# second-state/qwen3_asr_rs

Measured on NVIDIA H100. Metric: real-time factor (audio-sec/wall-sec) Qwen3-ASR-0.6B 30s clips, higher is better.
Workload: dtype f32 (bf16 weights, fp32-exact activations)

## Files before the change

qwen3_asr_rs_b200/csrc/attention_f32.cu:

```cuda
#include "internal.h"

namespace asrb {

namespace af32 {

static constexpr int QT = 32, KT = 64, THREADS = 128, PS = KT + 4;

template <int HD, bool OFF>
__global__ void __launch_bounds__(THREADS, 2) attn_f32_kernel(AttnParams p) {
    constexpr int NG = HD / 64;
    extern __shared__ __align__(16) float sm[];
    float* Qt = sm;
    float* Kt = Qt + HD * QT;
    float* Vs = Kt + HD * KT;
    float* Ps = Vs + KT * HD;
    const int seg = blockIdx.z, h = blockIdx.y;
    const int q0 = p.seg_q0[seg], len = p.seg_len[seg];
    const int pos0 = OFF ? p.seg_pos0[seg] : 0;
    const int nqt = (len + QT - 1) / QT;
    const int gkv = h / p.group;
    const int tid = threadIdx.x, tx = tid & 15, ty = tid >> 4;
    const float* kbase; const float* vbase;
    if (p.keys_in_rows) {
        kbase = p.k + (size_t)q0 * p.ldk + (size_t)gkv * p.head_stride;
        vbase = p.v + (size_t)q0 * p.ldk + (size_t)gkv * p.head_stride;
    } else {
        kbase = p.k + (size_t)seg * p.seg_stride + (size_t)gkv * p.head_stride;
        vbase = p.v + (size_t)seg * p.seg_stride + (size_t)gkv * p.head_stride;
    }
    const int npass = p.causal ? 2 : 1;
    for (int pass = 0; pass < npass; ++pass) {
    const int qtile = pass == 0 ? (int)blockIdx.x : nqt - 1 - (int)blockIdx.x;
    if (qtile >= nqt || qtile < 0 || (p.causal && pass == 0 && 2 * qtile >= nqt) || (pass == 1 && qtile <= (int)blockIdx.x)) continue;
    const int qt0 = qtile * QT;
    __syncthreads();
    {
        constexpr int NQ = QT * (HD / 4) / THREADS;
        float4 qr[NQ];
#pragma unroll
        for (int u = 0; u < NQ; ++u) {
            const int idx = tid + u * THREADS, r = idx % QT, c4 = idx / QT;
            qr[u] = make_float4(0.f, 0.f, 0.f, 0.f);
            if (qt0 + r < len) qr[u] = *reinterpret_cast<const float4*>(p.q + (size_t)(q0 + qt0 + r) * p.ldq + (size_t)h * HD + c4 * 4);
        }
#pragma unroll
        for (int u = 0; u < NQ; ++u) {
            const int idx = tid + u * THREADS, r = idx % QT, c4 = idx / QT;
            Qt[(c4 * 4 + 0) * QT + r] = qr[u].x; Qt[(c4 * 4 + 1) * QT + r] = qr[u].y;
            Qt[(c4 * 4 + 2) * QT + r] = qr[u].z; Qt[(c4 * 4 + 3) * QT + r] = qr[u].w;
        }
    }
    float o[4][NG][4];
#pragma unroll
    for (int i = 0; i < 4; ++i)
#pragma unroll
        for (int gq = 0; gq < NG; ++gq) { o[i][gq][0] = o[i][gq][1] = o[i][gq][2] = o[i][gq][3] = 0.f; }
    float m_run[4], l_run[4];
#pragma unroll
    for (int i = 0; i < 4; ++i) { m_run[i] = -INFINITY; l_run[i] = 0.f; }
    const int kend = p.causal ? pos0 + min(len, qt0 + QT) : len;
    const float div = sqrtf((float)HD);

    for (int kt0 = 0; kt0 < kend; kt0 += KT) {
        __syncthreads();
        constexpr int NLD = KT * (HD / 4) / THREADS, LB = 8;
        static_assert(NLD % LB == 0, "tile load batches");
#pragma unroll
        for (int b0 = 0; b0 < NLD; b0 += LB) {
            float4 kr[LB];
#pragma unroll
            for (int u = 0; u < LB; ++u) {
                const int idx = tid + (b0 + u) * THREADS, r = idx % KT, c4 = idx / KT;
                kr[u] = make_float4(0.f, 0.f, 0.f, 0.f);
                if (kt0 + r < kend) kr[u] = *reinterpret_cast<const float4*>(kbase + (size_t)(kt0 + r) * p.ldk + c4 * 4);
            }
#pragma unroll
            for (int u = 0; u < LB; ++u) {
                const int idx = tid + (b0 + u) * THREADS, r = idx % KT, c4 = idx / KT;
                Kt[(c4 * 4 + 0) * KT + r] = kr[u].x; Kt[(c4 * 4 + 1) * KT + r] = kr[u].y;
                Kt[(c4 * 4 + 2) * KT + r] = kr[u].z; Kt[(c4 * 4 + 3) * KT + r] = kr[u].w;
            }
        }
#pragma unroll
        for (int b0 = 0; b0 < NLD; b0 += LB) {
            float4 vr[LB];
#pragma unroll
            for (int u = 0; u < LB; ++u) {
                const int idx = tid + (b0 + u) * THREADS, r = idx / (HD / 4), c4 = idx - r * (HD / 4);
                vr[u] = make_float4(0.f, 0.f, 0.f, 0.f);
                if (kt0 + r < kend) vr[u] = *reinterpret_cast<const float4*>(vbase + (size_t)(kt0 + r) * p.ldk + c4 * 4);
            }
#pragma unroll
            for (int u = 0; u < LB; ++u) {
                const int idx = tid + (b0 + u) * THREADS, r = idx / (HD / 4), c4 = idx - r * (HD / 4);
                *reinterpret_cast<float4*>(Vs + r * HD + c4 * 4) = vr[u];
            }
        }
        __syncthreads();
        float s[4][4];
#pragma unroll
        for (int i = 0; i < 4; ++i) { s[i][0] = s[i][1] = s[i][2] = s[i][3] = 0.f; }
#pragma unroll 8
        for (int d = 0; d < HD; ++d) {
            const float4 a = *reinterpret_cast<const float4*>(Qt + d * QT + ty * 4);
            const float4 b = *reinterpret_cast<const float4*>(Kt + d * KT + tx * 4);
            s[0][0] = fmaf(a.x, b.x, s[0][0]); s[0][1] = fmaf(a.x, b.y, s[0][1]); s[0][2] = fmaf(a.x, b.z, s[0][2]); s[0][3] = fmaf(a.x, b.w, s[0][3]);
            s[1][0] = fmaf(a.y, b.x, s[1][0]); s[1][1] = fmaf(a.y, b.y, s[1][1]); s[1][2] = fmaf(a.y, b.z, s[1][2]); s[1][3] = fmaf(a.y, b.w, s[1][3]);
            s[2][0] = fmaf(a.z, b.x, s[2][0]); s[2][1] = fmaf(a.z, b.y, s[2][1]); s[2][2] = fmaf(a.z, b.z, s[2][2]); s[2][3] = fmaf(a.z, b.w, s[2][3]);
            s[3][0] = fmaf(a.w, b.x, s[3][0]); s[3][1] = fmaf(a.w, b.y, s[3][1]); s[3][2] = fmaf(a.w, b.z, s[3][2]); s[3][3] = fmaf(a.w, b.w, s[3][3]);
        }
#pragma unroll
        for (int i = 0; i < 4; ++i) {
            const int r = qt0 + ty * 4 + i;
            float tmax = -INFINITY;
#pragma unroll
            for (int j = 0; j < 4; ++j) {
                const int col = kt0 + tx * 4 + j;
                const bool valid = (r < len) && (col < pos0 + len) && (!p.causal || col <= pos0 + r);
                const float v = valid ? s[i][j] / div : -INFINITY;
                s[i][j] = v;
                tmax = fmaxf(tmax, v);
            }
#pragma unroll
            for (int off = 1; off < 16; off <<= 1) tmax = fmaxf(tmax, __shfl_xor_sync(0xffffffffu, tmax, off));
            const float m_new = fmaxf(m_run[i], tmax);
            const float corr = (m_new == -INFINITY) ? 1.f : expf(m_run[i] - m_new);
            m_run[i] = m_new;
            float psum = 0.f;
            float4 pv;
            pv.x = (m_new == -INFINITY) ? 0.f : expf(s[i][0] - m_new);
            pv.y = (m_new == -INFINITY) ? 0.f : expf(s[i][1] - m_new);
            pv.z = (m_new == -INFINITY) ? 0.f : expf(s[i][2] - m_new);
            pv.w = (m_new == -INFINITY) ? 0.f : expf(s[i][3] - m_new);
            psum = (pv.x + pv.y) + (pv.z + pv.w);
#pragma unroll
            for (int off = 1; off < 16; off <<= 1) psum += __shfl_xor_sync(0xffffffffu, psum, off);
            l_run[i] = l_run[i] * corr + psum;
#pragma unroll
            for (int gq = 0; gq < NG; ++gq) { o[i][gq][0] *= corr; o[i][gq][1] *= corr; o[i][gq][2] *= corr; o[i][gq][3] *= corr; }
            *reinterpret_cast<float4*>(Ps + (ty * 4 + i) * PS + tx * 4) = pv;
        }
        __syncwarp();
#pragma unroll 4
        for (int j = 0; j < KT; ++j) {
            float a[4];
#pragma unroll
            for (int i = 0; i < 4; ++i) a[i] = Ps[(ty * 4 + i) * PS + j];
#pragma unroll
            for (int gq = 0; gq < NG; ++gq) {
                const float4 b = *reinterpret_cast<const float4*>(Vs + j * HD + gq * 64 + tx * 4);
#pragma unroll
                for (int i = 0; i < 4; ++i) {
                    o[i][gq][0] = fmaf(a[i], b.x, o[i][gq][0]); o[i][gq][1] = fmaf(a[i], b.y, o[i][gq][1]);
                    o[i][gq][2] = fmaf(a[i], b.z, o[i][gq][2]); o[i][gq][3] = fmaf(a[i], b.w, o[i][gq][3]);
                }
            }
        }
        __syncwarp();
    }
#pragma unroll
    for (int i = 0; i < 4; ++i) {
        const int r = qt0 + ty * 4 + i;
        if (r >= len) continue;
        const float inv = 1.0f / l_run[i];
        const size_t base = (size_t)(q0 + r) * p.ldo + (size_t)h * HD;
#pragma unroll
        for (int gq = 0; gq < NG; ++gq)
#pragma unroll
            for (int e = 0; e < 4; ++e) store_split3(p.out_s3, p.plane_stride, base + gq * 64 + tx * 4 + e, o[i][gq][e] * inv);
    }
    }
}

template <int HD> static size_t smem_bytes() { return (size_t)(HD * QT + HD * KT + KT * HD + QT * PS) * sizeof(float); }

}

bool launch_attention_f32(const AttnParams& p, int hd, cudaStream_t st) {
    using namespace af32;
    if (p.nseg <= 0 || p.max_len <= 0) return true;
    if ((p.ldq % 4) || (p.ldk % 4) || (p.head_stride % 4) || (p.seg_stride % 4)) return false;
    const int nqt_max = (p.max_len + QT - 1) / QT;
    dim3 grid(p.causal ? (nqt_max + 1) / 2 : nqt_max, p.nheads, p.nseg);
    auto run = [&](auto kern, size_t smem) {
        ASRB_CUDA_CHECK(cudaFuncSetAttribute(kern, cudaFuncAttributeMaxDynamicSharedMemorySize, (int)smem));
        kern<<<grid, THREADS, smem, st>>>(p);
    };
    const bool off = p.seg_pos0 != nullptr;
    if (off && !p.causal) return false;
    if (hd == 64) run(off ? attn_f32_kernel<64, true> : attn_f32_kernel<64, false>, smem_bytes<64>());
    else if (hd == 128) run(off ? attn_f32_kernel<128, true> : attn_f32_kernel<128, false>, smem_bytes<128>());
    else return false;
    ASRB_CUDA_CHECK(cudaGetLastError());
    return true;
}

}
```

qwen3_asr_rs_b200/csrc/common.cuh:

```cuda
#pragma once
#include <cuda_runtime.h>
#include <cuda_bf16.h>
#include <stdint.h>
#include <stdexcept>
#include <string>

namespace asrb {

struct Error : public std::runtime_error {
    int code;
    Error(int c, const std::string& m) : std::runtime_error(m), code(c) {}
};

#define ASRB_CUDA_CHECK(expr)                                                              \
    do {                                                                                   \
        cudaError_t _e = (expr);                                                           \
        if (_e != cudaSuccess)                                                             \
            throw ::asrb::Error(2, std::string(#expr) + " failed: " + cudaGetErrorString(_e) + \
                                       " (" __FILE__ ":" + std::to_string(__LINE__) + ")"); \
    } while (0)

#define ASRB_REQUIRE(cond, code, msg)                                          \
    do {                                                                       \
        if (!(cond)) throw ::asrb::Error((code), std::string(msg));            \
    } while (0)

typedef __nv_bfloat16 bf16;

__device__ __forceinline__ float bf16_bits_to_f32(uint32_t bits16) { return __uint_as_float(bits16 << 16); }
__device__ __forceinline__ float bf16_lo(uint32_t packed) { return __uint_as_float(packed << 16); }
__device__ __forceinline__ float bf16_hi(uint32_t packed) { return __uint_as_float(packed & 0xffff0000u); }

struct Split3 { bf16 hi, mid, lo; };
__device__ __forceinline__ Split3 split3(float x) {
    Split3 s;
    s.hi = __float2bfloat16_rn(x);
    float r = x - __bfloat162float(s.hi);
    s.mid = __float2bfloat16_rn(r);
    r = r - __bfloat162float(s.mid);
    s.lo = __float2bfloat16_rn(r);
    return s;
}
__device__ __forceinline__ void store_split3(bf16* base, size_t plane_stride, size_t idx, float x) {
    Split3 s = split3(x);
    base[idx] = s.hi;
    base[plane_stride + idx] = s.mid;
    base[2 * plane_stride + idx] = s.lo;
}
__device__ __forceinline__ float load_split3(const bf16* base, size_t plane_stride, size_t idx, int nplanes) {
    float v = __bfloat162float(base[idx]);
    if (nplanes > 1) v += __bfloat162float(base[plane_stride + idx]);
    if (nplanes > 2) v += __bfloat162float(base[2 * plane_stride + idx]);
    return v;
}

__device__ __forceinline__ float gelu_erf(float x) {
    return 0.5f * x * (1.0f + erff(x * 0.70710678118654752440f));
}
__device__ __forceinline__ float silu(float x) { return x / (1.0f + expf(-x)); }

__device__ __forceinline__ float warp_sum(float v) {
#pragma unroll
    for (int o = 16; o > 0; o >>= 1) v += __shfl_xor_sync(0xffffffffu, v, o);
    return v;
}
__device__ __forceinline__ float warp_max(float v) {
#pragma unroll
    for (int o = 16; o > 0; o >>= 1) v = fmaxf(v, __shfl_xor_sync(0xffffffffu, v, o));
    return v;
}
__device__ __forceinline__ float block_sum(float v, float* scratch) {
    int lane = threadIdx.x & 31, w = threadIdx.x >> 5, nw = (blockDim.x + 31) >> 5;
    v = warp_sum(v);
    __syncthreads();
    if (lane == 0) scratch[w] = v;
    __syncthreads();
    float r = (lane < nw) ? scratch[lane] : 0.f;
    r = warp_sum(r);
    return r;
}
__device__ __forceinline__ float block_max(float v, float* scratch) {
    int lane = threadIdx.x & 31, w = threadIdx.x >> 5, nw = (blockDim.x + 31) >> 5;
    v = warp_max(v);
    __syncthreads();
    if (lane == 0) scratch[w] = v;
    __syncthreads();
    float r = (lane < nw) ? scratch[lane] : -INFINITY;
    r = warp_max(r);
    return r;
}

__device__ __forceinline__ float lse_rescale(float s, float m, float M) { return m == M ? s : s * expf(m - M); }
__device__ __forceinline__ void lse_fold(float v, int row, float& best_v, int& best_i, float& best_s) {
    if (v > best_v) { best_s = lse_rescale(best_s, best_v, v) + 1.f; best_v = v; best_i = row; }
    else best_s += expf(v - best_v);
}
__device__ __forceinline__ float lse_merge(float m, float s, float om, float os) {
    const float M = fmaxf(m, om);
    return lse_rescale(s, m, M) + lse_rescale(os, om, M);
}

constexpr int TK_MAX = 8;
struct TopK { float v[TK_MAX]; int i[TK_MAX]; };
__device__ __forceinline__ bool tk_before(float a, int ai, float b, int bi) { return a > b || (a == b && ai < bi); }
__device__ __forceinline__ void tk_init(TopK& t) {
#pragma unroll
    for (int j = 0; j < TK_MAX; ++j) { t.v[j] = -INFINITY; t.i[j] = 0x7fffffff; }
}
__device__ __forceinline__ void tk_insert(TopK& t, float v, int row) {
    if (!tk_before(v, row, t.v[TK_MAX - 1], t.i[TK_MAX - 1])) return;
#pragma unroll
    for (int j = 0; j < TK_MAX; ++j)
        if (tk_before(v, row, t.v[j], t.i[j])) { const float tv = t.v[j]; const int ti = t.i[j]; t.v[j] = v; t.i[j] = row; v = tv; row = ti; }
}
__device__ __forceinline__ void tk_merge(TopK& t, const TopK& u) {
#pragma unroll
    for (int j = 0; j < TK_MAX; ++j)
        if (!tk_before(t.v[j], t.i[j], u.v[TK_MAX - 1 - j], u.i[TK_MAX - 1 - j])) { t.v[j] = u.v[TK_MAX - 1 - j]; t.i[j] = u.i[TK_MAX - 1 - j]; }
#pragma unroll
    for (int d = TK_MAX / 2; d > 0; d >>= 1)
#pragma unroll
        for (int j = 0; j < TK_MAX; ++j)
            if ((j & d) == 0 && tk_before(t.v[j + d], t.i[j + d], t.v[j], t.i[j])) {
                const float tv = t.v[j]; const int ti = t.i[j];
                t.v[j] = t.v[j + d]; t.i[j] = t.i[j + d]; t.v[j + d] = tv; t.i[j + d] = ti;
            }
}
__device__ __forceinline__ void tk_merge_xor(TopK& t, int o) {
    TopK u;
#pragma unroll
    for (int j = 0; j < TK_MAX; ++j) { u.v[j] = __shfl_xor_sync(0xffffffffu, t.v[j], o); u.i[j] = __shfl_xor_sync(0xffffffffu, t.i[j], o); }
    tk_merge(t, u);
}
__device__ __forceinline__ void tk_store(const TopK& t, float* v, int* i) {
#pragma unroll
    for (int j = 0; j < TK_MAX; ++j) { v[j] = t.v[j]; i[j] = t.i[j]; }
}
__device__ __forceinline__ void tk_merge_from(TopK& t, const float* v, const int* i, bool l2) {
    TopK u;
#pragma unroll
    for (int j = 0; j < TK_MAX; ++j) { u.v[j] = l2 ? __ldcg(v + j) : v[j]; u.i[j] = l2 ? __ldcg(i + j) : i[j]; }
    tk_merge(t, u);
}
__device__ __forceinline__ void tk_write(const TopK& t, float lp, int* ids, float* lps) {
#pragma unroll
    for (int j = 0; j < TK_MAX; ++j) { ids[j] = t.i[j]; lps[j] = j == 0 ? lp : (t.v[j] - t.v[0]) + lp; }
}

struct SampleParams {
    float inv_t;
    uint32_t k0, k1;
};
__host__ __device__ __forceinline__ uint32_t philox4x32_10_x0(uint32_t c0, uint32_t c1, uint32_t c2, uint32_t c3, uint32_t k0, uint32_t k1) {
#pragma unroll
    for (int i = 0; i < 10; ++i) {
        if (i > 0) { k0 += 0x9E3779B9u; k1 += 0xBB67AE85u; }
        const uint64_t p0 = (uint64_t)0xD2511F53u * c0, p1 = (uint64_t)0xCD9E8D57u * c2;
        const uint32_t n0 = (uint32_t)(p1 >> 32) ^ c1 ^ k0, n2 = (uint32_t)(p0 >> 32) ^ c3 ^ k1;
        c0 = n0; c1 = (uint32_t)p1; c2 = n2; c3 = (uint32_t)p0;
    }
    return c0;
}
struct Draw {
    float inv_t; uint32_t k0, k1, n, r;
};
__device__ __forceinline__ Draw make_draw(const SampleParams* sp, int n, int r) {
    Draw d; d.inv_t = __ldg(&sp->inv_t); d.k0 = __ldg(&sp->k0); d.k1 = __ldg(&sp->k1); d.n = (uint32_t)n; d.r = (uint32_t)r;
    return d;
}
__device__ __forceinline__ float gumbel_noise(uint32_t x0) {
    const float u = (float)((x0 >> 8) | 1u) * 0x1p-24f;
    return -logf(-logf(u));
}
__device__ __forceinline__ float sample_key(const Draw& d, float l, int v) {
    return fmaf(l, d.inv_t, gumbel_noise(philox4x32_10_x0((uint32_t)v, d.n, d.r, 0u, d.k0, d.k1)));
}
template <bool LOGPROB>
__device__ __forceinline__ void sample_fold(const Draw& d, float l, int row, float& best_v, int& best_i, float& best_s, float& m,
                                            float& sel) {
    const float k = sample_key(d, l, row);
    if (k > best_v) { best_v = k; best_i = row; if constexpr (LOGPROB) sel = l; }
    if constexpr (LOGPROB) {
        if (l > m) { best_s = lse_rescale(best_s, m, l) + 1.f; m = l; }
        else best_s += expf(l - m);
    }
}
template <bool LOGPROB>
__device__ __forceinline__ void sample_merge_xor(int o, float& best_v, int& best_i, float& best_s, float& m, float& sel) {
    const float ov = __shfl_xor_sync(0xffffffffu, best_v, o); const int oi = __shfl_xor_sync(0xffffffffu, best_i, o);
    float osel = 0.f;
    if constexpr (LOGPROB) {
        osel = __shfl_xor_sync(0xffffffffu, sel, o);
        const float om = __shfl_xor_sync(0xffffffffu, m, o);
        best_s = lse_merge(m, best_s, om, __shfl_xor_sync(0xffffffffu, best_s, o));
        m = fmaxf(m, om);
    }
    if (ov > best_v || (ov == best_v && oi < best_i)) { best_v = ov; best_i = oi; if constexpr (LOGPROB) sel = osel; }
}

struct RepParams {
    float theta;
    int ngram;
};
struct RepBits {
    const uint32_t* hist; const uint32_t* ban; int w0; float theta;
};
__device__ __forceinline__ void rep_mark(const int* __restrict__ ids, int n, int N, int lo, int hi, uint32_t* hist,
                                         uint32_t* ban, int t, int nt) {
    const int w0 = lo >> 5;
    for (int i = t; i < n; i += nt) {
        const int v = __ldcg(ids + i);
        if (v >= lo && v < hi) atomicOr(hist + ((v >> 5) - w0), 1u << (v & 31));
        if (N >= 1 && i <= n - N) {
            bool match = true;
            for (int j = 0; j < N - 1 && match; ++j) match = __ldcg(ids + i + j) == __ldcg(ids + n - N + 1 + j);
            if (match) {
                const int u = __ldcg(ids + i + N - 1);
                if (u >= lo && u < hi) atomicOr(ban + ((u >> 5) - w0), 1u << (u & 31));
            }
        }
    }
}
__device__ __forceinline__ bool rep_logit(const RepBits& r, int v, float& l) {
    const int w = (v >> 5) - r.w0;
    const uint32_t bit = 1u << (v & 31);
    if (r.ban[w] & bit) { l = -INFINITY; return false; }
    if (r.hist[w] & bit) l = l < 0.f ? l * r.theta : l / r.theta;
    return true;
}
template <bool REP>
__device__ __forceinline__ bool rep_keep(const RepBits* r, int v, float& l) {
    if constexpr (REP) return rep_logit(*r, v, l);
    else return true;
}

__device__ __host__ __forceinline__ int float_to_ordered(float f) {
#ifdef __CUDA_ARCH__
    int i = __float_as_int(f);
#else
    int i; memcpy(&i, &f, 4);
#endif
    return i >= 0 ? i : i ^ 0x7fffffff;
}
__device__ __forceinline__ float ordered_to_float(int k) {
    int i = k >= 0 ? k : k ^ 0x7fffffff;
    return __int_as_float(i);
}

}
```

qwen3_asr_rs_b200/csrc/elementwise.cu:

```cuda
#include "internal.h"

namespace asrb {

__global__ void conv1_gelu_kernel(const float* __restrict__ mel, const int* __restrict__ chunk_clip,
                                  const int* __restrict__ chunk_f0, const int64_t* __restrict__ foff,
                                  const int64_t* __restrict__ frames, int n_mels, int W, int OH, int OW,
                                  const float* __restrict__ w, const float* __restrict__ bias, int dsh,
                                  int cpad, bf16* __restrict__ out, size_t plane_stride) {
    extern __shared__ float rows[];
    const int chunk = blockIdx.y, oh = blockIdx.x;
    const int clip = chunk_clip[chunk], f0 = chunk_f0[chunk];
    const int F = (int)frames[clip];
    const float* mp = mel + (size_t)n_mels * foff[clip];
    for (int idx = threadIdx.x; idx < 3 * (W + 2); idx += blockDim.x) {
        int kh = idx / (W + 2), wi = idx - kh * (W + 2);
        int h = 2 * oh + kh - 1, wcol = wi - 1;
        float v = 0.f;
        if (h >= 0 && h < n_mels && wcol >= 0 && wcol < W && f0 + wcol < F) v = mp[(size_t)h * F + f0 + wcol];
        rows[idx] = v;
    }
    __syncthreads();
    const int c = threadIdx.x;
    if (c >= dsh) return;
    float wk[9];
#pragma unroll
    for (int i = 0; i < 9; ++i) wk[i] = w[c * 9 + i];
    const float bc = bias ? bias[c] : 0.f;
    const int Hh = OH / 2 + (OH & 1), Wh = (OW + 1) / 2;
    for (int ow = 0; ow < OW; ++ow) {
        float acc = bc;
#pragma unroll
        for (int kh = 0; kh < 3; ++kh)
#pragma unroll
            for (int kw = 0; kw < 3; ++kw) acc = fmaf(wk[kh * 3 + kw], rows[kh * (W + 2) + 2 * ow + kw], acc);
        float v = gelu_erf(acc);
        size_t pos = ((((size_t)chunk * 2 + (oh & 1)) * 2 + (ow & 1)) * Hh + (oh >> 1)) * Wh + (ow >> 1);
        store_split3(out, plane_stride, pos * cpad + c, v);
    }
}

void launch_conv1(const Model& m, const float* mel, const int* d_chunk_clip, const int* d_chunk_f0,
                  const int64_t* d_foff, const int64_t* d_frames, int n_chunks, bf16* out_s3,
                  size_t plane_stride, cudaStream_t st) {
    const Dims& d = m.d;
    int W = d.conv_w[0], OH = d.conv_h[1], OW = d.conv_w[1];
    dim3 grid(OH, n_chunks);
    int threads = ((d.c.downsample_hidden_size + 31) / 32) * 32;
    size_t smem = 3 * (W + 2) * sizeof(float);
    conv1_gelu_kernel<<<grid, threads, smem, st>>>(mel, d_chunk_clip, d_chunk_f0, d_foff, d_frames,
                                                   d.c.num_mel_bins, W, OH, OW, m.conv1_w, m.conv1_b,
                                                   d.c.downsample_hidden_size, d.cpad, out_s3, plane_stride);
    ASRB_CUDA_CHECK(cudaGetLastError());
}

__global__ void layernorm_s3_kernel(const float* __restrict__ x, const float* __restrict__ w,
                                    const float* __restrict__ b, int dim, float eps, bf16* __restrict__ out,
                                    size_t plane_stride) {
    __shared__ float red[32];
    const size_t row = blockIdx.x;
    const float* xr = x + row * dim;
    float s = 0.f;
    for (int i = threadIdx.x; i < dim; i += blockDim.x) s += xr[i];
    const float mean = block_sum(s, red) / dim;
    float v = 0.f;
    for (int i = threadIdx.x; i < dim; i += blockDim.x) { float dlt = xr[i] - mean; v = fmaf(dlt, dlt, v); }
    const float var = block_sum(v, red) / dim;
    const float rstd = 1.0f / sqrtf(var + eps);
    for (int i = threadIdx.x; i < dim; i += blockDim.x)
        store_split3(out, plane_stride, row * dim + i, (xr[i] - mean) * rstd * w[i] + b[i]);
}
__global__ void rmsnorm_s3_kernel(const float* __restrict__ x, const float* __restrict__ w, int dim, float eps,
                                  bf16* __restrict__ out, size_t plane_stride) {
    __shared__ float red[32];
    const size_t row = blockIdx.x;
    const float* xr = x + row * dim;
    float s = 0.f;
    for (int i = threadIdx.x; i < dim; i += blockDim.x) s = fmaf(xr[i], xr[i], s);
    const float var = block_sum(s, red) / dim;
    const float r = 1.0f / sqrtf(var + eps);
    for (int i = threadIdx.x; i < dim; i += blockDim.x)
        store_split3(out, plane_stride, row * dim + i, (xr[i] * r) * w[i]);
}
void launch_layernorm_s3(const float* x, const float* w, const float* b, int rows, int dim, float eps,
                         bf16* out_s3, size_t plane_stride, cudaStream_t st) {
    if (rows <= 0) return;
    layernorm_s3_kernel<<<rows, 128, 0, st>>>(x, w, b, dim, eps, out_s3, plane_stride);
    ASRB_CUDA_CHECK(cudaGetLastError());
}
void launch_rmsnorm_s3(const float* x, const float* w, int rows, int dim, float eps, bf16* out_s3,
                       size_t plane_stride, cudaStream_t st) {
    if (rows <= 0) return;
    rmsnorm_s3_kernel<<<rows, 128, 0, st>>>(x, w, dim, eps, out_s3, plane_stride);
    ASRB_CUDA_CHECK(cudaGetLastError());
}

__global__ void embed_inject_kernel(const bf16* __restrict__ embed, int hidden, const int* __restrict__ ids,
                                    const int* __restrict__ audio_row, const float* __restrict__ audio,
                                    float* __restrict__ out) {
    const size_t row = blockIdx.x;
    const int ar = audio_row[row];
    float* o = out + row * hidden;
    if (ar >= 0) {
        const float* a = audio + (size_t)ar * hidden;
        for (int i = threadIdx.x; i < hidden; i += blockDim.x) o[i] = a[i];
    } else {
        const bf16* e = embed + (size_t)ids[row] * hidden;
        for (int i = threadIdx.x; i < hidden; i += blockDim.x) o[i] = __bfloat162float(e[i]);
    }
}
void launch_embed_inject(const bf16* embed, int hidden, const int* d_ids, const int* d_audio_row,
                         const float* audio, int rows, float* out, cudaStream_t st) {
    if (rows <= 0) return;
    embed_inject_kernel<<<rows, 256, 0, st>>>(embed, hidden, d_ids, d_audio_row, audio, out);
    ASRB_CUDA_CHECK(cudaGetLastError());
}

template <bool FAN>
__global__ void qk_norm_rope_kernel(const float* __restrict__ qkv, const int* __restrict__ row_seq,
                                    const int* __restrict__ row_pos, const float* __restrict__ qnorm,
                                    const float* __restrict__ knorm, float eps,
                                    const float* __restrict__ rope_cos, const float* __restrict__ rope_sin,
                                    int nq, int nkv, int hd, float* __restrict__ q_out,
                                    float* __restrict__ kcache, float* __restrict__ vcache,
                                    size_t cache_seq_stride, int max_ctx, FanOut fan) {
    extern __shared__ float sh[];
    float* ys = sh;
    float* red = sh + hd;
    const size_t row = blockIdx.x;
    const int head = blockIdx.y, d = threadIdx.x;
    const int qkv_dim = (nq + 2 * nkv) * hd;
    const float x = qkv[row * qkv_dim + (size_t)head * hd + d];
    const int seq = row_seq[row], pos = row_pos[row];
    const int nfan = FAN && pos < fan.P[seq] ? fan.n[seq] : 0;
    const int* fslots = FAN ? fan.slots + fan.off[seq] : nullptr;
    if (head >= nq + nkv) {
        const size_t o = ((size_t)(head - nq - nkv) * max_ctx + pos) * hd + d;
        vcache[seq * cache_seq_stride + o] = x;
        for (int j = 0; j < nfan; ++j) vcache[(size_t)fslots[j] * cache_seq_stride + o] = x;
        return;
    }
    const float* nw = head < nq ? qnorm : knorm;
    const float var = block_sum(x * x, red) / hd;
    const float y = (x * (1.0f / sqrtf(var + eps))) * nw[d];
    ys[d] = y;
    __syncthreads();
    const int half = hd / 2;
    const float rot = d < half ? -ys[d + half] : ys[d - half];
    const float c = rope_cos[(size_t)pos * half + (d % half)], s = rope_sin[(size_t)pos * half + (d % half)];
    const float o = y * c + rot * s;
    if (head < nq) q_out[row * ((size_t)nq * hd) + (size_t)head * hd + d] = o;
    else {
        const size_t ko = ((size_t)(head - nq) * max_ctx + pos) * hd + d;
        kcache[seq * cache_seq_stride + ko] = o;
        for (int j = 0; j < nfan; ++j) kcache[(size_t)fslots[j] * cache_seq_stride + ko] = o;
    }
}
void launch_qk_norm_rope(const float* qkv, int rows, const int* d_row_seq, const int* d_row_pos,
                         const float* qnorm, const float* knorm, float eps, const float* rope_cos,
                         const float* rope_sin, int nq, int nkv, int hd, float* q_out, float* kcache,
                         float* vcache, size_t cache_seq_stride, int max_ctx, cudaStream_t st, const FanOut* fan) {
    if (rows <= 0) return;
    dim3 grid(rows, nq + 2 * nkv);
    const size_t smem = (hd + 32) * sizeof(float);
    if (fan) qk_norm_rope_kernel<true><<<grid, hd, smem, st>>>(qkv, d_row_seq, d_row_pos, qnorm, knorm, eps, rope_cos, rope_sin,
                                                               nq, nkv, hd, q_out, kcache, vcache, cache_seq_stride, max_ctx, *fan);
    else qk_norm_rope_kernel<false><<<grid, hd, smem, st>>>(qkv, d_row_seq, d_row_pos, qnorm, knorm, eps, rope_cos, rope_sin,
                                                            nq, nkv, hd, q_out, kcache, vcache, cache_seq_stride, max_ctx, FanOut{});
    ASRB_CUDA_CHECK(cudaGetLastError());
}

}
```

qwen3_asr_rs_b200/csrc/gemm_tc.cu:

```cuda
#include <cuda.h>
#include <algorithm>
#include <cstring>
#include <map>
#include <tuple>
#include "internal.h"
#include "epilogue.cuh"
#include "wgmma.cuh"

namespace asrb {
namespace tc {

static constexpr int BM = 128, BN = 128, BK = 64, STAGES = 3;
static constexpr int TILE_A_BYTES = BM * BK * 2;
static constexpr int TILE_B_BYTES = BN * BK * 2;
static constexpr int STAGE_BYTES = 3 * TILE_A_BYTES + TILE_B_BYTES;
static constexpr int NTHREADS = 384;
static constexpr int CONS_WARPS = 8;
static constexpr int SLAB_LD = 40;
static constexpr int CH = 4;

struct ConvGeom { int OH, OW, box_h, tiles_per_chunk, kblk_per_tap, a_box_bytes; };

template <int A_MODE, int EPI_MODE>
__global__ void __launch_bounds__(NTHREADS, 1)
gemm_tc_kernel(const __grid_constant__ CUtensorMap mapA, const __grid_constant__ CUtensorMap mapB,
               int M, int N, int K, int nplanes, int tiles_m, int tiles_n, int splits, ConvGeom cg, GemmEpi E) {
    extern __shared__ __align__(1024) uint8_t smem_raw[];
    uint8_t* smem = reinterpret_cast<uint8_t*>((reinterpret_cast<uintptr_t>(smem_raw) + 1023) & ~(uintptr_t)1023);
    uint64_t* full = reinterpret_cast<uint64_t*>(smem + STAGES * STAGE_BYTES);
    uint64_t* empty = full + STAGES;
    float* epi_slab = reinterpret_cast<float*>(smem + STAGES * STAGE_BYTES + 256);
    const int warp = threadIdx.x >> 5, lane = threadIdx.x & 31;
    const int num_kb = K / BK / splits;
    const int n_items = tiles_m * tiles_n * splits;

    if (threadIdx.x == 0) {
        for (int i = 0; i < STAGES; ++i) { mbar_init(&full[i], 1); mbar_init(&empty[i], CONS_WARPS); }
        asm volatile("fence.mbarrier_init.release.cluster;" ::: "memory");
        asm volatile("prefetch.tensormap [%0];" ::"l"(&mapA) : "memory");
        asm volatile("prefetch.tensormap [%0];" ::"l"(&mapB) : "memory");
    }
    __syncthreads();

    auto item_coords = [&](int item, int& n0, int& m0, int& chunk, int& oh0, int& z) {
        const int nt = item % tiles_n; int rest = item / tiles_n;
        const int mt = rest % tiles_m; z = rest / tiles_m;
        n0 = nt * BN; m0 = mt * BM; chunk = 0; oh0 = 0;
        if (A_MODE == 1) { chunk = mt / cg.tiles_per_chunk; oh0 = (mt % cg.tiles_per_chunk) * cg.box_h; }
    };

    if (warp == 0 && lane == 0) {
        const uint32_t a_bytes = (A_MODE == 0) ? (uint32_t)TILE_A_BYTES : (uint32_t)cg.a_box_bytes;
        const uint32_t stage_tx = (uint32_t)nplanes * a_bytes + (uint32_t)TILE_B_BYTES;
        uint32_t kg = 0;
        for (int item = blockIdx.x; item < n_items; item += gridDim.x) {
            int n0, m0, chunk, oh0, z;
            item_coords(item, n0, m0, chunk, oh0, z);
            const int kb0 = z * num_kb;
            for (int kb = 0; kb < num_kb; ++kb, ++kg) {
                const int s = kg % STAGES; const uint32_t par = (kg / STAGES) & 1;
                mbar_wait(&empty[s], par ^ 1);
                uint8_t* st = smem + s * STAGE_BYTES;
                mbar_expect_tx(&full[s], stage_tx);
                if (A_MODE == 0) {
                    for (int p = 0; p < nplanes; ++p) tma_load_3d(st + p * TILE_A_BYTES, &mapA, (kb0 + kb) * BK, m0, p, &full[s]);
                } else {
                    const int tap = kb / cg.kblk_per_tap, cb = kb % cg.kblk_per_tap;
                    const int kh = tap / 3, kw = tap % 3;
                    const int ph = (kh == 1) ? 0 : 1, pw = (kw == 1) ? 0 : 1;
                    const int h = oh0 + (kh == 0 ? -1 : 0), w = (kw == 0 ? -1 : 0);
                    for (int p = 0; p < nplanes; ++p)
                        tma_load_5d(st + p * TILE_A_BYTES, &mapA, cb * BK, w, h, (chunk * 2 + ph) * 2 + pw, p, &full[s]);
                }
                tma_load_2d(st + 3 * TILE_A_BYTES, &mapB, (kb0 + kb) * BK, n0, &full[s]);
            }
        }
    } else if (warp >= 4) {
        const int half = (warp >> 2) - 1, q = warp & 3;
        const int cw = warp - 4;
        float acc[64], sum[64];
#pragma unroll
        for (int j = 0; j < 64; ++j) acc[j] = 0.f;
        uint32_t kg = 0;
        for (int item = blockIdx.x; item < n_items; item += gridDim.x) {
            int n0, m0, chunk, oh0, z;
            item_coords(item, n0, m0, chunk, oh0, z);
#pragma unroll
            for (int j = 0; j < 64; ++j) sum[j] = 0.f;
            consume_k_blocks<STAGES, STAGE_BYTES, TILE_A_BYTES, BK, CH>(smem, full, empty, half, lane, num_kb, nplanes, kg, acc, sum);
            float* slab = epi_slab + cw * (16 * SLAB_LD);
            const int lr = lane >> 3, lc = (lane & 7) * 4;
#pragma unroll
            for (int g = 0; g < BN / 32; ++g) {
                stage_slab<SLAB_LD>(slab, sum, g, lane);
                const int n = n0 + g * 32 + lc;
                const bool ncol = n < N;
                const float4 bias4 = ncol ? epi_bias4<EPI_MODE>(E, n) : make_float4(0.f, 0.f, 0.f, 0.f);
                float4 v[4]; long long mr[4]; EpiIn in[4];
#pragma unroll
                for (int i = 0; i < 4; ++i) {
                    const int rr = half * 64 + q * 16 + 4 * i + lr;
                    v[i] = *reinterpret_cast<const float4*>(slab + (4 * i + lr) * SLAB_LD + lc);
                    long long m = -1;
                    if (A_MODE == 0) { if (m0 + rr < M) m = m0 + rr + (long long)z * M; }
                    else {
                        const int oh = oh0 + rr / cg.OW, ow = rr % cg.OW;
                        if (rr < cg.box_h * cg.OW && oh < cg.OH) m = ((long long)chunk * cg.OH + oh) * cg.OW + ow;
                    }
                    mr[i] = (m >= 0 && ncol) ? m : -1;
                    if (mr[i] >= 0) in[i] = epi_fetch4<EPI_MODE>(E, N, (int)mr[i], n);
                }
#pragma unroll
                for (int i = 0; i < 4; ++i)
                    if (mr[i] >= 0) epi_store4<EPI_MODE>(E, N, (int)mr[i], n, v[i], bias4, in[i]);
                __syncwarp();
            }
        }
    }
}

template <int MODE>
__global__ void __launch_bounds__(256) splitk_reduce_kernel(const float* __restrict__ ws, int S, int M, int N, GemmEpi E) {
    const int n8 = N / 8;
    const int idx = blockIdx.x * blockDim.x + threadIdx.x;
    if (idx >= M * n8) return;
    const int m = idx / n8, n = (idx - m * n8) * 8;
    float v[8];
#pragma unroll
    for (int i = 0; i < 8; ++i) v[i] = 0.f;
    for (int sp = 0; sp < S; ++sp) {
        const float* src = ws + ((size_t)sp * M + m) * N + n;
        const float4 a = *reinterpret_cast<const float4*>(src), b = *reinterpret_cast<const float4*>(src + 4);
        v[0] += a.x; v[1] += a.y; v[2] += a.z; v[3] += a.w; v[4] += b.x; v[5] += b.y; v[6] += b.z; v[7] += b.w;
    }
    epi_store8<MODE>(E, N, m, n, v);
}

typedef CUresult (*EncodeTiledFn)(CUtensorMap*, CUtensorMapDataType, cuuint32_t, void*, const cuuint64_t*, const cuuint64_t*,
                                  const cuuint32_t*, const cuuint32_t*, CUtensorMapInterleave, CUtensorMapSwizzle,
                                  CUtensorMapL2promotion, CUtensorMapFloatOOBfill);
static EncodeTiledFn get_encode() {
    static EncodeTiledFn fn = nullptr;
    if (!fn) {
        void* p = nullptr;
        cudaDriverEntryPointQueryResult qr;
        ASRB_CUDA_CHECK(cudaGetDriverEntryPoint("cuTensorMapEncodeTiled", &p, cudaEnableDefault, &qr));
        ASRB_REQUIRE(p != nullptr && qr == cudaDriverEntryPointSuccess, ASRB_ERR_CUDA, "cuTensorMapEncodeTiled unavailable");
        fn = (EncodeTiledFn)p;
    }
    return fn;
}
static CUtensorMap make_map(const void* base, int rank, const cuuint64_t* dims, const cuuint64_t* strides_bytes, const cuuint32_t* box) {
    CUtensorMap m;
    cuuint32_t estr[5] = {1, 1, 1, 1, 1};
    CUresult r = get_encode()(&m, CU_TENSOR_MAP_DATA_TYPE_BFLOAT16, (cuuint32_t)rank, const_cast<void*>(base), dims, strides_bytes, box,
                              estr, CU_TENSOR_MAP_INTERLEAVE_NONE, CU_TENSOR_MAP_SWIZZLE_128B, CU_TENSOR_MAP_L2_PROMOTION_L2_128B,
                              CU_TENSOR_MAP_FLOAT_OOB_FILL_NONE);
    if (r != CUDA_SUCCESS) throw Error(ASRB_ERR_CUDA, "cuTensorMapEncodeTiled failed with code " + std::to_string((int)r));
    return m;
}

struct MapKey {
    const void* base; int rank; cuuint64_t d[5]; cuuint64_t s[4]; cuuint32_t b[5];
    bool operator<(const MapKey& o) const { return memcmp(this, &o, sizeof(MapKey)) < 0; }
};
static const CUtensorMap& cached_map(const void* base, int rank, const cuuint64_t* dims, const cuuint64_t* strides_bytes, const cuuint32_t* box) {
    static thread_local std::map<MapKey, CUtensorMap> cache;
    MapKey k;
    memset(&k, 0, sizeof(k));
    k.base = base; k.rank = rank;
    for (int i = 0; i < rank; ++i) { k.d[i] = dims[i]; k.b[i] = box[i]; }
    for (int i = 0; i + 1 < rank; ++i) k.s[i] = strides_bytes[i];
    auto it = cache.find(k);
    if (it == cache.end()) {
        if (cache.size() > 4096) cache.clear();
        it = cache.emplace(k, make_map(base, rank, dims, strides_bytes, box)).first;
    }
    return it->second;
}

static int sm_count() {
    int dev = 0, n = 132;
    if (cudaGetDevice(&dev) == cudaSuccess) cudaDeviceGetAttribute(&n, cudaDevAttrMultiProcessorCount, dev);
    return n;
}
static size_t smem_bytes() { return (size_t)STAGES * STAGE_BYTES + 1024 + 256 + CONS_WARPS * 16 * SLAB_LD * 4; }

}

const CUtensorMap& tc_cached_map(const void* base, int rank, const cuuint64_t* dims, const cuuint64_t* strides_bytes,
                                 const cuuint32_t* box) {
    return tc::cached_map(base, rank, dims, strides_bytes, box);
}

GemmPlan plan_gemm_tc(const GemmA& A, int N, const GemmEpi& E, int sms) {
    using namespace tc;
    GemmPlan p;
    if (A.K % BK != 0 || A.M <= 0 || N <= 0 || N % 8 != 0) return p;
    if (A.nplanes < 1 || A.nplanes > 3) return p;
    if (A.mode == A_PLAIN) {
        if (A.plane_stride % 8 != 0 && A.nplanes > 1) return p;
        if (E.mode != EPI_PLAIN && E.mode != EPI_SWIGLU && E.mode != EPI_CONVOUT) return p;
        p.tiles_n = (N + BN - 1) / BN; p.tiles_m = (A.M + BM - 1) / BM;
        const int tiles = p.tiles_n * p.tiles_m, kblocks = A.K / BK;
        if ((E.mode == EPI_PLAIN || E.mode == EPI_CONVOUT) && E.splitk_ws && tiles <= 64 && (size_t)4 * A.M * N <= SPLITK_WS_FLOATS) {
            for (int sp = 4; sp >= 2; --sp)
                if (kblocks % sp == 0 && kblocks / sp >= 6 && tiles * sp <= sms + sms / 12) { p.splits = sp; break; }
        }
    } else {
        if (A.cpad % BK != 0 || A.OW > BM || A.OW <= 0 || A.OH <= 0) return p;
        if (E.mode != EPI_CONV_PARITY && E.mode != EPI_CONV_FEAT) return p;
        p.box_h = std::min(A.OH, BM / A.OW);
        p.tiles_n = (N + BN - 1) / BN;
        p.tiles_m = (A.M / (A.OH * A.OW)) * ((A.OH + p.box_h - 1) / p.box_h);
    }
    p.grid = std::min(p.tiles_m * p.tiles_n * p.splits, sms);
    p.tc = p.grid > 0;
    return p;
}

bool launch_gemm_tc(const GemmA& A, const bf16* W, int N, const GemmEpi& Ein, cudaStream_t st) {
    using namespace tc;
    const GemmEpi& E = Ein;
    static const bool time_all = getenv("ASRB_GEMM_TIME") != nullptr;
    struct Timer {
        bool on; cudaEvent_t e0, e1; int M, N, K, mode; cudaStream_t st;
        Timer(bool o, int M_, int N_, int K_, int mode_, cudaStream_t s) : on(o), M(M_), N(N_), K(K_), mode(mode_), st(s) {
            if (on) { cudaEventCreate(&e0); cudaEventCreate(&e1); cudaEventRecord(e0, st); }
        }
        ~Timer() {
            if (!on) return;
            cudaEventRecord(e1, st); cudaEventSynchronize(e1);
            float ms = 0.f; cudaEventElapsedTime(&ms, e0, e1);
            fprintf(stderr, "[gemm_tc time] M=%d N=%d K=%d epi=%d %.1f us\n", M, N, K, mode, ms * 1000.f);
            cudaEventDestroy(e0); cudaEventDestroy(e1);
        }
    } timer(time_all, A.M, N, A.K, E.mode, st);
    const GemmPlan pl = plan_gemm_tc(A, N, E, sm_count());
    if (!pl.tc) return false;
    if ((reinterpret_cast<uintptr_t>(A.a) & 15) || (reinterpret_cast<uintptr_t>(W) & 15)) return false;
    cuuint64_t bd[2] = {(cuuint64_t)A.K, (cuuint64_t)N};
    cuuint64_t bs[1] = {(cuuint64_t)A.K * 2};
    cuuint32_t bb[2] = {(cuuint32_t)BK, (cuuint32_t)BN};
    const CUtensorMap mapB = cached_map(W, 2, bd, bs, bb);
    ConvGeom cg{};
    const size_t smem = smem_bytes();
    const int tiles_m = pl.tiles_m, tiles_n = pl.tiles_n;
    if (A.mode == A_PLAIN) {
        cuuint64_t ad[3] = {(cuuint64_t)A.K, (cuuint64_t)A.M, (cuuint64_t)3};
        cuuint64_t as[2] = {(cuuint64_t)A.lda * 2, (cuuint64_t)A.plane_stride * 2};
        cuuint32_t ab[3] = {(cuuint32_t)BK, (cuuint32_t)BM, 1};
        const CUtensorMap mapA = cached_map(A.a, 3, ad, as, ab);
        if (pl.splits > 1) {
            GemmEpi P;
            P.out_f32 = E.splitk_ws; P.ldo = N;
            ASRB_CUDA_CHECK(cudaFuncSetAttribute(gemm_tc_kernel<0, EPI_PLAIN>, cudaFuncAttributeMaxDynamicSharedMemorySize, (int)smem));
            gemm_tc_kernel<0, EPI_PLAIN><<<pl.grid, NTHREADS, smem, st>>>(mapA, mapB, A.M, N, A.K, A.nplanes, tiles_m, tiles_n, pl.splits, cg, P);
            const int work = A.M * (N / 8);
            if (E.mode == EPI_PLAIN) splitk_reduce_kernel<EPI_PLAIN><<<(work + 255) / 256, 256, 0, st>>>(E.splitk_ws, pl.splits, A.M, N, E);
            else splitk_reduce_kernel<EPI_CONVOUT><<<(work + 255) / 256, 256, 0, st>>>(E.splitk_ws, pl.splits, A.M, N, E);
            ASRB_CUDA_CHECK(cudaGetLastError());
            if (E.extra_launches) *E.extra_launches += 1;
            return true;
        }
#define ASRB_TC_LAUNCH(AM, EM)                                                                                         \
    {                                                                                                                  \
        ASRB_CUDA_CHECK(cudaFuncSetAttribute(gemm_tc_kernel<AM, EM>, cudaFuncAttributeMaxDynamicSharedMemorySize, (int)smem)); \
        gemm_tc_kernel<AM, EM><<<pl.grid, NTHREADS, smem, st>>>(mapA, mapB, A.M, N, A.K, A.nplanes, tiles_m, tiles_n, 1, cg, E); \
    }
        if (E.mode == EPI_PLAIN) ASRB_TC_LAUNCH(0, EPI_PLAIN)
        else if (E.mode == EPI_SWIGLU) ASRB_TC_LAUNCH(0, EPI_SWIGLU)
        else ASRB_TC_LAUNCH(0, EPI_CONVOUT)
    } else {
        const int chunks = A.M / (A.OH * A.OW);
        cg.OH = A.OH; cg.OW = A.OW; cg.box_h = pl.box_h;
        cg.tiles_per_chunk = (A.OH + cg.box_h - 1) / cg.box_h; cg.kblk_per_tap = A.cpad / BK;
        cg.a_box_bytes = A.OW * cg.box_h * BK * 2;
        cuuint64_t ad[5] = {(cuuint64_t)A.cpad, (cuuint64_t)A.Wh, (cuuint64_t)A.Hh, (cuuint64_t)chunks * 4, 3};
        cuuint64_t as[4] = {(cuuint64_t)A.cpad * 2, (cuuint64_t)A.Wh * A.cpad * 2, (cuuint64_t)A.Hh * A.Wh * A.cpad * 2,
                            (cuuint64_t)A.plane_stride * 2};
        cuuint32_t ab[5] = {(cuuint32_t)BK, (cuuint32_t)A.OW, (cuuint32_t)cg.box_h, 1, 1};
        const CUtensorMap mapA = cached_map(A.a, 5, ad, as, ab);
        if (E.mode == EPI_CONV_PARITY) ASRB_TC_LAUNCH(1, EPI_CONV_PARITY)
        else ASRB_TC_LAUNCH(1, EPI_CONV_FEAT)
#undef ASRB_TC_LAUNCH
    }
    ASRB_CUDA_CHECK(cudaGetLastError());
    return true;
}

}
```

Baseline: 333.0.

## Enable programmatic dependent launch and prefetch GEMM weights before waiting

Switches most kernel launches to cudaLaunchKernelEx with programmatic stream serialization and adds griddepcontrol.wait at kernel entry, so each kernel's launch and prologue can overlap the tail of the previous kernel. In the tensor-core GEMM, the producer issues TMA loads of the first weight stages before the dependency wait, since weights do not depend on the prior kernel. No kernel calls an explicit launch_dependents trigger, so the overlap relies on the implicit trigger at grid completion. Correctness depends on every PDL-launched kernel waiting before it reads predecessor outputs.

```diff
diff --git a/qwen3_asr_rs_b200/csrc/attention_f32.cu b/qwen3_asr_rs_b200/csrc/attention_f32.cu
--- a/qwen3_asr_rs_b200/csrc/attention_f32.cu
+++ b/qwen3_asr_rs_b200/csrc/attention_f32.cu
@@ -14,6 +14,7 @@
     float* Kt = Qt + HD * QT;
     float* Vs = Kt + HD * KT;
     float* Ps = Vs + KT * HD;
+    pdl_wait();
     const int seg = blockIdx.z, h = blockIdx.y;
     const int q0 = p.seg_q0[seg], len = p.seg_len[seg];
     const int pos0 = OFF ? p.seg_pos0[seg] : 0;
@@ -184,7 +185,7 @@
     dim3 grid(p.causal ? (nqt_max + 1) / 2 : nqt_max, p.nheads, p.nseg);
     auto run = [&](auto kern, size_t smem) {
         ASRB_CUDA_CHECK(cudaFuncSetAttribute(kern, cudaFuncAttributeMaxDynamicSharedMemorySize, (int)smem));
-        kern<<<grid, THREADS, smem, st>>>(p);
+        launch_pdl(kern, grid, THREADS, smem, st, p);
     };
     const bool off = p.seg_pos0 != nullptr;
     if (off && !p.causal) return false;
diff --git a/qwen3_asr_rs_b200/csrc/common.cuh b/qwen3_asr_rs_b200/csrc/common.cuh
--- a/qwen3_asr_rs_b200/csrc/common.cuh
+++ b/qwen3_asr_rs_b200/csrc/common.cuh
@@ -52,6 +52,19 @@
     if (nplanes > 1) v += __bfloat162float(base[plane_stride + idx]);
     if (nplanes > 2) v += __bfloat162float(base[2 * plane_stride + idx]);
     return v;
+}
+
+__device__ __forceinline__ void pdl_wait() { asm volatile("griddepcontrol.wait;" ::: "memory"); }
+
+template <typename... KArgs, typename... Args>
+inline void launch_pdl(void (*kernel)(KArgs...), dim3 grid, dim3 block, size_t smem, cudaStream_t st, Args&&... args) {
+    cudaLaunchAttribute attr[1];
+    attr[0].id = cudaLaunchAttributeProgrammaticStreamSerialization;
+    attr[0].val.programmaticStreamSerializationAllowed = 1;
+    cudaLaunchConfig_t cfg = {};
+    cfg.gridDim = grid; cfg.blockDim = block; cfg.dynamicSmemBytes = smem; cfg.stream = st;
+    cfg.attrs = attr; cfg.numAttrs = 1;
+    ASRB_CUDA_CHECK(cudaLaunchKernelEx(&cfg, kernel, std::forward<Args>(args)...));
 }
 
 __device__ __forceinline__ float gelu_erf(float x) {
diff --git a/qwen3_asr_rs_b200/csrc/elementwise.cu b/qwen3_asr_rs_b200/csrc/elementwise.cu
--- a/qwen3_asr_rs_b200/csrc/elementwise.cu
+++ b/qwen3_asr_rs_b200/csrc/elementwise.cu
@@ -8,6 +8,7 @@
                                   const float* __restrict__ w, const float* __restrict__ bias, int dsh,
                                   int cpad, bf16* __restrict__ out, size_t plane_stride) {
     extern __shared__ float rows[];
+    pdl_wait();
     const int chunk = blockIdx.y, oh = blockIdx.x;
     const int clip = chunk_clip[chunk], f0 = chunk_f0[chunk];
     const int F = (int)frames[clip];
@@ -47,9 +48,8 @@
     dim3 grid(OH, n_chunks);
     int threads = ((d.c.downsample_hidden_size + 31) / 32) * 32;
     size_t smem = 3 * (W + 2) * sizeof(float);
-    conv1_gelu_kernel<<<grid, threads, smem, st>>>(mel, d_chunk_clip, d_chunk_f0, d_foff, d_frames,
-                                                   d.c.num_mel_bins, W, OH, OW, m.conv1_w, m.conv1_b,
-                                                   d.c.downsample_hidden_size, d.cpad, out_s3, plane_stride);
+    launch_pdl(conv1_gelu_kernel, grid, threads, smem, st, mel, d_chunk_clip, d_chunk_f0, d_foff, d_frames, d.c.num_mel_bins, W,
+               OH, OW, (const float*)m.conv1_w, (const float*)m.conv1_b, d.c.downsample_hidden_size, d.cpad, out_s3, plane_stride);
     ASRB_CUDA_CHECK(cudaGetLastError());
 }
 
@@ -57,6 +57,7 @@
                                     const float* __restrict__ b, int dim, float eps, bf16* __restrict__ out,
                                     size_t plane_stride) {
     __shared__ float red[32];
+    pdl_wait();
     const size_t row = blockIdx.x;
     const float* xr = x + row * dim;
     float s = 0.f;
@@ -72,6 +73,7 @@
 __global__ void rmsnorm_s3_kernel(const float* __restrict__ x, const float* __restrict__ w, int dim, float eps,
                                   bf16* __restrict__ out, size_t plane_stride) {
     __shared__ float red[32];
+    pdl_wait();
     const size_t row = blockIdx.x;
     const float* xr = x + row * dim;
     float s = 0.f;
@@ -84,19 +86,20 @@
 void launch_layernorm_s3(const float* x, const float* w, const float* b, int rows, int dim, float eps,
                          bf16* out_s3, size_t plane_stride, cudaStream_t st) {
     if (rows <= 0) return;
-    layernorm_s3_kernel<<<rows, 128, 0, st>>>(x, w, b, dim, eps, out_s3, plane_stride);
+    launch_pdl(layernorm_s3_kernel, rows, 128, 0, st, x, w, b, dim, eps, out_s3, plane_stride);
     ASRB_CUDA_CHECK(cudaGetLastError());
 }
 void launch_rmsnorm_s3(const float* x, const float* w, int rows, int dim, float eps, bf16* out_s3,
                        size_t plane_stride, cudaStream_t st) {
     if (rows <= 0) return;
-    rmsnorm_s3_kernel<<<rows, 128, 0, st>>>(x, w, dim, eps, out_s3, plane_stride);
+    launch_pdl(rmsnorm_s3_kernel, rows, 128, 0, st, x, w, dim, eps, out_s3, plane_stride);
     ASRB_CUDA_CHECK(cudaGetLastError());
 }
 
 __global__ void embed_inject_kernel(const bf16* __restrict__ embed, int hidden, const int* __restrict__ ids,
                                     const int* __restrict__ audio_row, const float* __restrict__ audio,
                                     float* __restrict__ out) {
+    pdl_wait();
     const size_t row = blockIdx.x;
     const int ar = audio_row[row];
     float* o = out + row * hidden;
@@ -111,7 +114,7 @@
 void launch_embed_inject(const bf16* embed, int hidden, const int* d_ids, const int* d_audio_row,
                          const float* audio, int rows, float* out, cudaStream_t st) {
     if (rows <= 0) return;
-    embed_inject_kernel<<<rows, 256, 0, st>>>(embed, hidden, d_ids, d_audio_row, audio, out);
+    launch_pdl(embed_inject_kernel, rows, 256, 0, st, embed, hidden, d_ids, d_audio_row, audio, out);
     ASRB_CUDA_CHECK(cudaGetLastError());
 }
 
@@ -126,6 +129,7 @@
     extern __shared__ float sh[];
     float* ys = sh;
     float* red = sh + hd;
+    pdl_wait();
     const size_t row = blockIdx.x;
     const int head = blockIdx.y, d = threadIdx.x;
     const int qkv_dim = (nq + 2 * nkv) * hd;
@@ -162,10 +166,9 @@
     if (rows <= 0) return;
     dim3 grid(rows, nq + 2 * nkv);
     const size_t smem = (hd + 32) * sizeof(float);
-    if (fan) qk_norm_rope_kernel<true><<<grid, hd, smem, st>>>(qkv, d_row_seq, d_row_pos, qnorm, knorm, eps, rope_cos, rope_sin,
-                                                               nq, nkv, hd, q_out, kcache, vcache, cache_seq_stride, max_ctx, *fan);
-    else qk_norm_rope_kernel<false><<<grid, hd, smem, st>>>(qkv, d_row_seq, d_row_pos, qnorm, knorm, eps, rope_cos, rope_sin,
-                                                            nq, nkv, hd, q_out, kcache, vcache, cache_seq_stride, max_ctx, FanOut{});
+    launch_pdl(fan ? qk_norm_rope_kernel<true> : qk_norm_rope_kernel<false>, grid, hd, smem, st, qkv, d_row_seq, d_row_pos,
+               qnorm, knorm, eps, rope_cos, rope_sin, nq, nkv, hd, q_out, kcache, vcache, cache_seq_stride, max_ctx,
+               fan ? *fan : FanOut{});
     ASRB_CUDA_CHECK(cudaGetLastError());
 }
 
diff --git a/qwen3_asr_rs_b200/csrc/gemm_tc.cu b/qwen3_asr_rs_b200/csrc/gemm_tc.cu
--- a/qwen3_asr_rs_b200/csrc/gemm_tc.cu
+++ b/qwen3_asr_rs_b200/csrc/gemm_tc.cu
@@ -49,9 +49,20 @@
         if (A_MODE == 1) { chunk = mt / cg.tiles_per_chunk; oh0 = (mt % cg.tiles_per_chunk) * cg.box_h; }
     };
 
+    const uint32_t a_bytes = (A_MODE == 0) ? (uint32_t)TILE_A_BYTES : (uint32_t)cg.a_box_bytes;
+    const uint32_t stage_tx = (uint32_t)nplanes * a_bytes + (uint32_t)TILE_B_BYTES;
+    const int pre_kb = blockIdx.x < n_items ? min(STAGES, num_kb) : 0;
+    if (warp == 0 && lane == 0 && pre_kb > 0) {
+        int n0, m0, chunk, oh0, z;
+        item_coords(blockIdx.x, n0, m0, chunk, oh0, z);
+        for (int kb = 0; kb < pre_kb; ++kb) {
+            mbar_expect_tx(&full[kb], stage_tx);
+            tma_load_2d(smem + kb * STAGE_BYTES + 3 * TILE_A_BYTES, &mapB, (z * num_kb + kb) * BK, n0, &full[kb]);
+        }
+    }
+    pdl_wait();
+
     if (warp == 0 && lane == 0) {
-        const uint32_t a_bytes = (A_MODE == 0) ? (uint32_t)TILE_A_BYTES : (uint32_t)cg.a_box_bytes;
-        const uint32_t stage_tx = (uint32_t)nplanes * a_bytes + (uint32_t)TILE_B_BYTES;
         uint32_t kg = 0;
         for (int item = blockIdx.x; item < n_items; item += gridDim.x) {
             int n0, m0, chunk, oh0, z;
@@ -59,9 +70,9 @@
             const int kb0 = z * num_kb;
             for (int kb = 0; kb < num_kb; ++kb, ++kg) {
                 const int s = kg % STAGES; const uint32_t par = (kg / STAGES) & 1;
-                mbar_wait(&empty[s], par ^ 1);
+                const bool pre = kg < (uint32_t)pre_kb;
                 uint8_t* st = smem + s * STAGE_BYTES;
-                mbar_expect_tx(&full[s], stage_tx);
+                if (!pre) { mbar_wait(&empty[s], par ^ 1); mbar_expect_tx(&full[s], stage_tx); }
                 if (A_MODE == 0) {
                     for (int p = 0; p < nplanes; ++p) tma_load_3d(st + p * TILE_A_BYTES, &mapA, (kb0 + kb) * BK, m0, p, &full[s]);
                 } else {
@@ -72,7 +83,7 @@
                     for (int p = 0; p < nplanes; ++p)
                         tma_load_5d(st + p * TILE_A_BYTES, &mapA, cb * BK, w, h, (chunk * 2 + ph) * 2 + pw, p, &full[s]);
                 }
-                tma_load_2d(st + 3 * TILE_A_BYTES, &mapB, (kb0 + kb) * BK, n0, &full[s]);
+                if (!pre) tma_load_2d(st + 3 * TILE_A_BYTES, &mapB, (kb0 + kb) * BK, n0, &full[s]);
             }
         }
     } else if (warp >= 4) {
@@ -121,6 +132,7 @@
 
 template <int MODE>
 __global__ void __launch_bounds__(256) splitk_reduce_kernel(const float* __restrict__ ws, int S, int M, int N, GemmEpi E) {
+    pdl_wait();
     const int n8 = N / 8;
     const int idx = blockIdx.x * blockDim.x + threadIdx.x;
     if (idx >= M * n8) return;
@@ -255,10 +267,11 @@
             GemmEpi P;
             P.out_f32 = E.splitk_ws; P.ldo = N;
             ASRB_CUDA_CHECK(cudaFuncSetAttribute(gemm_tc_kernel<0, EPI_PLAIN>, cudaFuncAttributeMaxDynamicSharedMemorySize, (int)smem));
-            gemm_tc_kernel<0, EPI_PLAIN><<<pl.grid, NTHREADS, smem, st>>>(mapA, mapB, A.M, N, A.K, A.nplanes, tiles_m, tiles_n, pl.splits, cg, P);
+            launch_pdl(gemm_tc_kernel<0, EPI_PLAIN>, pl.grid, NTHREADS, smem, st, mapA, mapB, A.M, N, A.K, A.nplanes, tiles_m, tiles_n,
+                       pl.splits, cg, P);
             const int work = A.M * (N / 8);
-            if (E.mode == EPI_PLAIN) splitk_reduce_kernel<EPI_PLAIN><<<(work + 255) / 256, 256, 0, st>>>(E.splitk_ws, pl.splits, A.M, N, E);
-            else splitk_reduce_kernel<EPI_CONVOUT><<<(work + 255) / 256, 256, 0, st>>>(E.splitk_ws, pl.splits, A.M, N, E);
+            launch_pdl(E.mode == EPI_PLAIN ? splitk_reduce_kernel<EPI_PLAIN> : splitk_reduce_kernel<EPI_CONVOUT>, (work + 255) / 256, 256, 0,
+                       st, (const float*)E.splitk_ws, pl.splits, A.M, N, E);
             ASRB_CUDA_CHECK(cudaGetLastError());
             if (E.extra_launches) *E.extra_launches += 1;
             return true;
@@ -266,7 +279,7 @@
 #define ASRB_TC_LAUNCH(AM, EM)                                                                                         \
     {                                                                                                                  \
         ASRB_CUDA_CHECK(cudaFuncSetAttribute(gemm_tc_kernel<AM, EM>, cudaFuncAttributeMaxDynamicSharedMemorySize, (int)smem)); \
-        gemm_tc_kernel<AM, EM><<<pl.grid, NTHREADS, smem, st>>>(mapA, mapB, A.M, N, A.K, A.nplanes, tiles_m, tiles_n, 1, cg, E); \
+        launch_pdl(gemm_tc_kernel<AM, EM>, pl.grid, NTHREADS, smem, st, mapA, mapB, A.M, N, A.K, A.nplanes, tiles_m, tiles_n, 1, cg, E); \
     }
         if (E.mode == EPI_PLAIN) ASRB_TC_LAUNCH(0, EPI_PLAIN)
         else if (E.mode == EPI_SWIGLU) ASRB_TC_LAUNCH(0, EPI_SWIGLU)
```

New measurement: 335.6, median of 6. Within noise of the previous version (+0.8%).
